# mworchel/svbrdf-estimation

Measured on AMD Instinct MI355X. Metric: rendered 256x256 patches/sec (fwd+bwd rendering loss), higher is better.
Workload: dtype f32

## Files before the change

### svbrdf_estimation_amd/csrc/svbrdf_kernels.hip

```cpp

#include <hip/hip_runtime.h>

#include <atomic>
#include <cstdint>
#include <cstdio>
#include <cstdlib>
#include <cmath>
#include <cstring>

#include "svbrdf_hip.h"

#ifndef SVBRDF_TU
#define SVBRDF_TU 2
#endif
#define SVBRDF_TU_MAIN (SVBRDF_TU == 0 || SVBRDF_TU == 2)
#define SVBRDF_TU_ADJOINT_PLAIN (SVBRDF_TU == 1 || SVBRDF_TU == 2)
#define SVBRDF_TU_ADJOINT_EXTRA (SVBRDF_TU == 3 || SVBRDF_TU == 2)
#define SVBRDF_TU_AUX (SVBRDF_TU == 4)

namespace {

constexpr int kThreads = 256;
constexpr int kLossThreads = 256;
constexpr float kPi = 3.14159274101257324219f;
constexpr float kMinDot = 0.001f;
constexpr float kMinRough = 0.001f;


__device__ __forceinline__ float dot3(float ax, float ay, float az, float bx, float by, float bz)
{
    const float p0 = ax * bx, p1 = ay * by, p2 = az * bz;
    return (p0 + p1) + p2;
}

__device__ __forceinline__ float fma_(float a, float b, float c) { return __builtin_fmaf(a, b, c); }
__device__ __forceinline__ float rcp_(float x) { return __builtin_amdgcn_rcpf(x); }
__device__ __forceinline__ float rsq_(float x) { return __builtin_amdgcn_rsqf(x); }
__device__ __forceinline__ float log2_(float x) { return __builtin_amdgcn_logf(x); }

#ifndef SVBRDF_SCALE_BLOCKS
#define SVBRDF_SCALE_BLOCKS 1024
#endif
#ifndef SVBRDF_TIMING
#define SVBRDF_TIMING 0
#endif
#ifndef SVBRDF_K3_MIN_WAVES
#define SVBRDF_K3_MIN_WAVES 4
#endif

struct Recip {
    float b, y;
};
__device__ __forceinline__ float div_rn(float a, const Recip &r)
{
    const float q = a * r.y;
    return fma_(fma_(-r.b, q, a), r.y, q);
}

__device__ __forceinline__ Recip length_rn(float x, float &seed)
{
    const float y = rsq_(x);
    const float g = x * y;
    seed = y;
    const float len = fma_(fma_(-g, g, x), 0.5f * y, g);
    const float e = fma_(-len, y, 1.0f);
    return Recip{len, fma_(e, y, y)};
}

struct VConst {
    float tiny;
    float pi, inv_pi;
    float ln2;
    float huge;
};
__device__ __forceinline__ float vreg(float c)
{
    asm volatile("" : "+v"(c));
    return c;
}
__device__ __forceinline__ VConst make_vconst()
{
    return VConst{vreg(kMinDot), vreg(kPi), vreg(1.0f / kPi), vreg(0.693147180559945309417f), vreg(1.0e30f)};
}


struct Geom {
    float wox, woy, woz;
    float wix, wiy, wiz;
    float hx, hy, hz;
    float p;
    float E[3];
};

__device__ __forceinline__ Geom geometry(const VConst &K, const float sc[9], float x, float y)
{
    Geom g;
    const float rcx = sc[0] - x, rcy = sc[1] - y, rcz = sc[2];
    const float rlx = sc[3] - x, rly = sc[4] - y, rlz = sc[5];
    float yc, yl, yh;
    const Recip ic = length_rn(dot3(rcx, rcy, rcz, rcx, rcy, rcz), yc);
    const Recip il = length_rn(dot3(rlx, rly, rlz, rlx, rly, rlz), yl);
    g.wox = div_rn(rcx, ic); g.woy = div_rn(rcy, ic); g.woz = div_rn(rcz, ic);
    g.wix = div_rn(rlx, il); g.wiy = div_rn(rly, il); g.wiz = div_rn(rlz, il);
    const float sx = g.wix + g.wox, sy = g.wiy + g.woy, sz = g.wiz + g.woz;
    const Recip ih = length_rn(dot3(sx, sy, sz, sx, sy, sz), yh);
    g.hx = div_rn(sx, ih); g.hy = div_rn(sy, ih); g.hz = div_rn(sz, ih);
    const float VH = fmaxf(fma_(g.wox, g.hx, fma_(g.woy, g.hy, g.woz * g.hz)), K.tiny);
    const float t = 1.0f - VH;
    const float t2 = t * t;
    g.p = (t2 * t2) * t;
    const float fall = yl * yl;
#pragma unroll
    for (int k = 0; k < 3; ++k) g.E[k] = sc[6 + k] * fall;
    return g;
}

struct Maps {
    float n[3], d[3], r[3], s[3];
};

struct Grad {
    float n[3], d[3], r[3], s[3];
};

struct MapK {
    float n[3];
    float A[3];
    float oA[3];
    float s[3], oms[3];
    float dpi[3];
    float r4m[3];
};

template <bool BWD>
__device__ __forceinline__ MapK prepare(const Maps &m)
{
    MapK k;
    constexpr float inv_pi = 1.0f / kPi;
#pragma unroll
    for (int c = 0; c < 3; ++c) {
        const float r = fmaxf(m.r[c], kMinRough);
        const float a = r * r;
        k.n[c] = m.n[c];
        k.A[c] = a * a;
        k.oA[c] = 1.0f - k.A[c];
        k.s[c] = m.s[c];
        k.oms[c] = 1.0f - m.s[c];
        k.dpi[c] = m.d[c] * inv_pi;
        if (BWD) k.r4m[c] = (m.r[c] >= kMinRough) ? 4.0f * (a * r) : 0.0f;
    }
    return k;
}

__device__ __forceinline__ bool tied_roughness(const Maps &m) { return m.r[0] == m.r[1] && m.r[1] == m.r[2]; }

struct Dots {
    float nh_raw, vn_raw, ln_raw;
    float NH, NH2, oN;
    float VN, LN;
    float VN2, LN2;
    float LNp;
};

__device__ __forceinline__ Dots dots(const VConst &K, const Geom &g, const MapK &m)
{
    Dots d;
    d.nh_raw = dot3(m.n[0], m.n[1], m.n[2], g.hx, g.hy, g.hz);
    d.vn_raw = fma_(g.wox, m.n[0], fma_(g.woy, m.n[1], g.woz * m.n[2]));
    d.ln_raw = fma_(g.wix, m.n[0], fma_(g.wiy, m.n[1], g.wiz * m.n[2]));
    d.NH = fmaxf(d.nh_raw, K.tiny);
    d.VN = fmaxf(d.vn_raw, K.tiny);
    d.LN = fmaxf(d.ln_raw, K.tiny);
    d.LNp = fmaxf(d.ln_raw, 0.0f);
    d.NH2 = d.NH * d.NH;
    d.oN = 1.0f - d.NH2;
    d.VN2 = d.VN * d.VN;
    d.LN2 = d.LN * d.LN;
    return d;
}

struct Lobe {
    float GD, KA, KV, KL, KN;
};

template <bool BWD>
__device__ __forceinline__ Lobe lobe(const VConst &K, float A, float oA, const Dots &d)
{
    Lobe l;
    const float yV = fma_(d.VN2, oA, A), yL = fma_(d.LN2, oA, A);
    const float iV = rsq_(yV), iL = rsq_(yL);
    const float sV = yV * iV, sL = yL * iL;
    const float PV = d.VN + sV, PL = d.LN + sL;
    const float PP = PV * PL;
    const float den_raw = fma_(d.NH2, A, d.oN);
    const float den = fmaxf(den_raw, K.tiny);
    const float pd = K.pi * den;
    const float Q = pd * den;
    const float R = rcp_(PP * Q);
    l.GD = A * R;
    if (BWD) {
        const float RQ = R * Q;
        const float tV = (RQ * PL) * l.GD;
        const float tL = (RQ * PV) * l.GD;
        l.KV = -tV * fma_(d.VN * oA, iV, 1.0f);
        l.KL = -tL * fma_(d.LN * oA, iL, 1.0f);
        const float Kden = (den_raw >= K.tiny) ? (-2.0f * l.GD) * ((R * PP) * pd) : 0.0f;
        const float hV = (1.0f - d.VN2) * iV, hL = (1.0f - d.LN2) * iL;
        l.KA = fma_(-0.5f, fma_(tV, hV, tL * hL), fma_(Kden, d.NH2, R));
        l.KN = -Kden * oA;
    }
    return l;
}

template <int NL, bool BWD>
__device__ __forceinline__ void shade(const VConst &K, const Geom &g, const MapK &m, const Dots &d, Lobe lb[NL],
                                      float F[3], float f[3], float rad[3])
{
#pragma unroll
    for (int l = 0; l < NL; ++l) lb[l] = lobe<BWD>(K, m.A[l], m.oA[l], d);
#pragma unroll
    for (int k = 0; k < 3; ++k) {
        F[k] = fma_(m.oms[k], g.p, m.s[k]);
        f[k] = fma_(F[k], lb[NL == 3 ? k : 0].GD - m.dpi[k], m.dpi[k]);
        rad[k] = f[k] * (g.E[k] * d.LNp);
    }
}

template <int NL, bool DEFER_D = false, bool DEFER_R = false>
__device__ __forceinline__ void shade_bwd(const VConst &K, const Geom &g, const MapK &m, const Dots &d, const Lobe lb[NL],
                                          const float F[3], const float f[3], const float g_rad[3], Grad &acc)
{
    float g_LNp, W[NL];
    const float inv_pi = K.inv_pi;
    const float omp = 1.0f - g.p;
#pragma unroll
    for (int k = 0; k < 3; ++k) {
        const Lobe &l = lb[NL == 3 ? k : 0];
        const float gE = g_rad[k] * g.E[k];
        const float g_f = gE * d.LNp;
        g_LNp = k == 0 ? gE * f[k] : fma_(gE, f[k], g_LNp);
        const float g_F = g_f * (l.GD - m.dpi[k]);
        acc.s[k] = fma_(g_F, omp, acc.s[k]);
        acc.d[k] = DEFER_D ? fma_(g_f, 1.0f - F[k], acc.d[k]) : fma_(g_f * (1.0f - F[k]), inv_pi, acc.d[k]);
        const float gGD = g_f * F[k];
        acc.r[k] = DEFER_R ? fma_(gGD, l.KA, acc.r[k]) : fma_(gGD * l.KA, m.r4m[k], acc.r[k]);
        if (NL == 3 || k == 0) W[NL == 3 ? k : 0] = gGD;
        else W[0] += gGD;
    }
    float g_VN = W[0] * lb[0].KV, g_LN = W[0] * lb[0].KL, sN = W[0] * lb[0].KN;
#pragma unroll
    for (int l = 1; l < NL; ++l) {
        g_VN = fma_(W[l], lb[l].KV, g_VN);
        g_LN = fma_(W[l], lb[l].KL, g_LN);
        sN = fma_(W[l], lb[l].KN, sN);
    }
    float g_NH = (sN * 2.0f) * d.NH;
    if (!(d.nh_raw >= K.tiny)) g_NH = 0.0f;
    if (!(d.vn_raw >= K.tiny)) g_VN = 0.0f;
    if (!(d.ln_raw >= K.tiny)) g_LN = 0.0f;
    if (!(d.ln_raw >= 0.0f)) g_LNp = 0.0f;
    const float gl = g_LN + g_LNp;
    acc.n[0] = fma_(g_NH, g.hx, fma_(g_VN, g.wox, fma_(gl, g.wix, acc.n[0])));
    acc.n[1] = fma_(g_NH, g.hy, fma_(g_VN, g.woy, fma_(gl, g.wiy, acc.n[1])));
    acc.n[2] = fma_(g_NH, g.hz, fma_(g_VN, g.woz, fma_(gl, g.wiz, acc.n[2])));
}


typedef float vec2f __attribute__((ext_vector_type(2)));
typedef float vec4f __attribute__((ext_vector_type(4)));
template <int VEC> struct VecT;
template <> struct VecT<1> { using type = float; };
template <> struct VecT<2> { using type = vec2f; };
template <> struct VecT<4> { using type = vec4f; };

template <int VEC, bool NT = false>
__device__ __forceinline__ void load_vec(const float *__restrict__ p, float out[VEC])
{
    using V = typename VecT<VEC>::type;
    const V v = NT ? __builtin_nontemporal_load(reinterpret_cast<const V *>(p)) : *reinterpret_cast<const V *>(p);
    const float *f = reinterpret_cast<const float *>(&v);
#pragma unroll
    for (int i = 0; i < VEC; ++i) out[i] = f[i];
}

template <int VEC, bool NT = false>
__device__ __forceinline__ void store_vec(float *__restrict__ p, const float in[VEC])
{
    using V = typename VecT<VEC>::type;
    V v;
    float *f = reinterpret_cast<float *>(&v);
#pragma unroll
    for (int i = 0; i < VEC; ++i) f[i] = in[i];
    if (NT) __builtin_nontemporal_store(v, reinterpret_cast<V *>(p));
    else *reinterpret_cast<V *>(p) = v;
}

template <int VEC, bool NT = false>
__device__ __forceinline__ void load_maps(const float *__restrict__ base, size_t plane, size_t pix,
                                          Maps m[VEC])
{
#pragma unroll
    for (int k = 0; k < 3; ++k) {
        float t[VEC];
        load_vec<VEC, NT>(base + (size_t)(0 + k) * plane + pix, t);
#pragma unroll
        for (int v = 0; v < VEC; ++v) m[v].n[k] = t[v];
        load_vec<VEC, NT>(base + (size_t)(3 + k) * plane + pix, t);
#pragma unroll
        for (int v = 0; v < VEC; ++v) m[v].d[k] = t[v];
        load_vec<VEC, NT>(base + (size_t)(6 + k) * plane + pix, t);
#pragma unroll
        for (int v = 0; v < VEC; ++v) m[v].r[k] = t[v];
        load_vec<VEC, NT>(base + (size_t)(9 + k) * plane + pix, t);
#pragma unroll
        for (int v = 0; v < VEC; ++v) m[v].s[k] = t[v];
    }
}

template <int VEC, bool NT = false>
__device__ __forceinline__ void store_grads(float *__restrict__ base, size_t plane, size_t pix,
                                            const Grad g[VEC])
{
#pragma unroll
    for (int k = 0; k < 3; ++k) {
        float t[VEC];
#pragma unroll
        for (int v = 0; v < VEC; ++v) t[v] = g[v].n[k];
        store_vec<VEC, NT>(base + (size_t)(0 + k) * plane + pix, t);
#pragma unroll
        for (int v = 0; v < VEC; ++v) t[v] = g[v].d[k];
        store_vec<VEC, NT>(base + (size_t)(3 + k) * plane + pix, t);
#pragma unroll
        for (int v = 0; v < VEC; ++v) t[v] = g[v].r[k];
        store_vec<VEC, NT>(base + (size_t)(6 + k) * plane + pix, t);
#pragma unroll
        for (int v = 0; v < VEC; ++v) t[v] = g[v].s[k];
        store_vec<VEC, NT>(base + (size_t)(9 + k) * plane + pix, t);
    }
}

#ifndef SVBRDF_K3_STORE_AUX
#define SVBRDF_K3_STORE_AUX 17
#endif
#ifndef SVBRDF_K3_LOAD_AUX
#define SVBRDF_K3_LOAD_AUX 0
#endif
struct PlaneBuf {
    __amdgpu_buffer_rsrc_t rsrc;
    unsigned lane_bytes;
    unsigned plane_bytes;
};
__device__ __forceinline__ PlaneBuf plane_buf(const float *item_base, int planes, size_t plane, size_t pix)
{
    PlaneBuf p;
    p.rsrc = __builtin_amdgcn_make_buffer_rsrc(const_cast<float *>(item_base), 0, (int)(planes * plane * sizeof(float)),
                                               0x00020000);
    p.lane_bytes = (unsigned)pix * 4u;
    p.plane_bytes = (unsigned)plane * 4u;
    return p;
}
__device__ __forceinline__ float plane_load(const PlaneBuf &p, int k)
{
    return __builtin_bit_cast(float, __builtin_amdgcn_raw_buffer_load_b32(p.rsrc, p.lane_bytes, k * p.plane_bytes, SVBRDF_K3_LOAD_AUX));
}
__device__ __forceinline__ void plane_store(const PlaneBuf &p, int k, float v)
{
    __builtin_amdgcn_raw_buffer_store_b32(__builtin_bit_cast(unsigned, v), p.rsrc, p.lane_bytes, k * p.plane_bytes,
                                          SVBRDF_K3_STORE_AUX);
}

__device__ __forceinline__ void load_maps_k3(const float *__restrict__ base, size_t plane, size_t pix, Maps &m)
{
    const PlaneBuf p = plane_buf(base, 12, plane, pix);
#pragma unroll
    for (int k = 0; k < 3; ++k) {
        m.n[k] = plane_load(p, 0 + k);
        m.d[k] = plane_load(p, 3 + k);
        m.r[k] = plane_load(p, 6 + k);
        m.s[k] = plane_load(p, 9 + k);
    }
}

__device__ __forceinline__ void store_grads_k3(float *__restrict__ base, size_t plane, size_t pix, const Grad &g)
{
    const PlaneBuf p = plane_buf(base, 12, plane, pix);
#pragma unroll
    for (int k = 0; k < 3; ++k) {
        plane_store(p, 0 + k, g.n[k]);
        plane_store(p, 3 + k, g.d[k]);
        plane_store(p, 6 + k, g.r[k]);
        plane_store(p, 9 + k, g.s[k]);
    }
}

__device__ __forceinline__ void zero_grad(Grad &g)
{
// ... 158 lines not shown

template <int VEC>
__global__ __launch_bounds__(kThreads) void k_render_fwd(const float *__restrict__ maps,
                                                         const float *__restrict__ scenes,
                                                         const float *__restrict__ xrow,
                                                         float *__restrict__ out, const int *__restrict__ offsets,
                                                         int shared, int S, int H, int W)
{
    render_fwd_body<VEC>(maps, scenes, xrow, out, offsets, shared != 0, S, H, W);
}

template <int VEC>
__global__ __launch_bounds__(kThreads) void k_render_fwd_inl([[maybe_unused]] const SceneBlock table,
                                                             const float *__restrict__ maps,
                                                             const float *__restrict__ xrow, float *__restrict__ out,
                                                             int shared, int S, int H, int W)
{
    const float *__restrict__ rows = (const float *)__builtin_amdgcn_kernarg_segment_ptr();
    render_fwd_body<VEC>(maps, rows, xrow, out, nullptr, shared != 0, S, H, W);
}

#ifndef SVBRDF_PHOTO_MIN_WAVES
#define SVBRDF_PHOTO_MIN_WAVES 4
#endif
#define SVBRDF_PHOTO_ATTRS __attribute__((amdgpu_waves_per_eu(SVBRDF_PHOTO_MIN_WAVES, 8)))
struct PhotoBlock {
    float v[SVBRDF_HOST_SCENES_MAX_ROWS * 9];
    float sigma[SVBRDF_HOST_SCENES_MAX_ROWS];
};

template <int VEC, int EPI>
__global__ __launch_bounds__(kThreads) SVBRDF_PHOTO_ATTRS void k_render_inputs(const float *__restrict__ maps,
                                                            const float *__restrict__ scenes,
                                                            const float *__restrict__ sigma, PhiloxKey key,
                                                            const float *__restrict__ xrow, float *__restrict__ out,
                                                            int S, int H, int W)
{
    render_fwd_body<VEC, EPI>(maps, scenes, xrow, out, nullptr, false, S, H, W, Epilogue{sigma, key});
}

template <int VEC, int EPI>
__global__ __launch_bounds__(kThreads) SVBRDF_PHOTO_ATTRS void k_render_inputs_inl([[maybe_unused]] const PhotoBlock table, PhiloxKey key,
                                                                const float *__restrict__ maps,
                                                                const float *__restrict__ xrow, float *__restrict__ out,
                                                                int S, int H, int W)
{
    const float *__restrict__ rows = (const float *)__builtin_amdgcn_kernarg_segment_ptr();
    render_fwd_body<VEC, EPI>(maps, rows, xrow, out, nullptr, false, S, H, W,
                              Epilogue{rows + SVBRDF_HOST_SCENES_MAX_ROWS * 9, key});
}

template <int VEC, int NL>
__device__ __forceinline__ void render_bwd_loop(const MapK mk[VEC], const float x[VEC], float y,
                                                const float *__restrict__ scp, const float *__restrict__ go,
                                                size_t plane, int S, Grad acc[VEC])
{
    const VConst K = make_vconst();
    for (int s = 0; s < S; ++s, scp += 9, go += 3 * plane) {
        float sc[9];
        load_scene(scp, sc);
        float gr[3][VEC];
#pragma unroll
        for (int k = 0; k < 3; ++k) load_vec<VEC, true>(go + (size_t)k * plane, gr[k]);
#pragma unroll
        for (int v = 0; v < VEC; ++v) {
            const Geom g = geometry(K, sc, x[v], y);
            const Dots d = dots(K, g, mk[v]);
            Lobe lb[NL];
            float F[3], f[3], rad[3];
            shade<NL, true>(K, g, mk[v], d, lb, F, f, rad);
            const float g_rad[3] = {gr[0][v], gr[1][v], gr[2][v]};
            shade_bwd<NL>(K, g, mk[v], d, lb, F, f, g_rad, acc[v]);
        }
    }
}

template <int VEC>
__device__ __forceinline__ void render_bwd_body(const float *__restrict__ maps, const float *__restrict__ scenes,
                                                const float *__restrict__ xrow, const float *__restrict__ grad_out,
                                                float *__restrict__ grad_maps, const int *__restrict__ offsets,
                                                bool shared, int S, int H, int W)
{
    const size_t plane = (size_t)H * W;
    const size_t pix = ((size_t)blockIdx.x * kThreads + threadIdx.x) * VEC;
    const int b = blockIdx.y;
    if (pix >= plane) return;
    MapK mk[VEC];
    bool tied = true;
    {
        Maps m[VEC];
        load_maps<VEC, true>(maps + (size_t)b * 12 * plane, plane, pix, m);
#pragma unroll
        for (int v = 0; v < VEC; ++v) {
            mk[v] = prepare<true>(m[v]);
            tied = tied && tied_roughness(m[v]);
        }
    }
    float x[VEC], y;
    pixel_coords<VEC>(xrow, pix, W, x, y);
    Grad acc[VEC];
#pragma unroll
    for (int v = 0; v < VEC; ++v) zero_grad(acc[v]);
    size_t first = (size_t)b * S;
    if (offsets) {
        first = (size_t)offsets[b];
        S = offsets[b + 1] - offsets[b];
    }
    const float *__restrict__ scp = scenes + (shared ? 0 : first * 9);
    const float *__restrict__ go = grad_out + first * 3 * plane + pix;
    if (__all(tied)) render_bwd_loop<VEC, 1>(mk, x, y, scp, go, plane, S, acc);
    else render_bwd_loop<VEC, 3>(mk, x, y, scp, go, plane, S, acc);
    store_grads<VEC, true>(grad_maps + (size_t)b * 12 * plane, plane, pix, acc);
}

template <int VEC>
__global__ __launch_bounds__(kThreads) void k_render_bwd(const float *__restrict__ maps,
                                                         const float *__restrict__ scenes,
                                                         const float *__restrict__ xrow,
                                                         const float *__restrict__ grad_out,
                                                         float *__restrict__ grad_maps, const int *__restrict__ offsets,
                                                         int shared, int S, int H, int W)
{
    render_bwd_body<VEC>(maps, scenes, xrow, grad_out, grad_maps, offsets, shared != 0, S, H, W);
}

template <int VEC>
__global__ __launch_bounds__(kThreads) void k_render_bwd_inl([[maybe_unused]] const SceneBlock table,
                                                             const float *__restrict__ maps,
                                                             const float *__restrict__ xrow,
                                                             const float *__restrict__ grad_out,
                                                             float *__restrict__ grad_maps, int shared, int S, int H, int W)
{
    const float *__restrict__ rows = (const float *)__builtin_amdgcn_kernarg_segment_ptr();
    render_bwd_body<VEC>(maps, rows, xrow, grad_out, grad_maps, nullptr, shared != 0, S, H, W);
}

__device__ __forceinline__ float wave_sum(float v)
{
#pragma unroll
    for (int off = 32; off > 0; off >>= 1) v += __shfl_xor(v, off, 64);
    return v;
}

constexpr int kLossSlots = 64;
constexpr int kLossCountShift = 48;
constexpr unsigned long long kLossSumMask = (1ULL << kLossCountShift) - 1;
constexpr unsigned long long kLossTicketMask = 0xffffffffULL;
constexpr unsigned long long kLossNonFiniteFlag = 1ULL << 32;

template <int NL, bool WITH_GRAD, int DEFER = 0>
__device__ __forceinline__ void loss_pixel_scene(const VConst &K, const Geom &g, const MapK &mi,
                                                 const MapK &mt, float eps, float inv_count, float &lsum, Grad &acc)
{
    float rt[3];
    {
        const Dots dt = dots(K, g, mt);
        Lobe lt[NL];
        float Ft[3], ft[3];
        shade<NL, false>(K, g, mt, dt, lt, Ft, ft, rt);
    }
    const Dots di = dots(K, g, mi);
    Lobe li[NL];
    float Fi[3], fi[3], ri[3], g_rad[3];
    shade<NL, WITH_GRAD>(K, g, mi, di, li, Fi, fi, ri);
    {
        constexpr float c = 9.765625e-04f;
        const float ec = eps * c, nc = inv_count * c;
        float b[3], bt[3], ib[3];
#pragma unroll
        for (int k = 0; k < 3; ++k) { b[k] = fma_(ri[k], c, ec); bt[k] = fma_(rt[k], c, ec); }
        {
            const float P = b[0] * b[1];
            const float r = rcp_(P * b[2]);
            const float t = r * b[2];
            ib[0] = t * b[1]; ib[1] = t * b[0]; ib[2] = r * P;
        }
#pragma unroll
        for (int k = 0; k < 3; ++k) {
            const float lg = (b[k] != bt[k]) ? log2_(bt[k] * ib[k]) : 0.0f;
            lsum += fabsf(lg);
            const float mag = (lg != 0.0f) ? nc * ib[k] : 0.0f;
            g_rad[k] = -__builtin_bit_cast(float, __builtin_bit_cast(unsigned, mag) | (__builtin_bit_cast(unsigned, lg) & 0x80000000u));
        }
    }
    if (WITH_GRAD) shade_bwd<NL, (DEFER & 1) != 0, (DEFER & 2) != 0>(K, g, mi, di, li, Fi, fi, g_rad, acc);
}

template <bool WITH_GRAD, int DEFER = 0>
__device__ __forceinline__ void loss_pixel_scene_by_channel(const VConst &K, const Geom &g, const MapK &mi, const MapK &mt,
                                                            float eps, float inv_count, float &lsum, Grad &acc)
{
    const Dots dt = dots(K, g, mt);
    const Dots di = dots(K, g, mi);
    constexpr float c = 9.765625e-04f;
    const float ec = eps * c, nc = inv_count * c;
    const float omp = 1.0f - g.p;
    float g_LNp = 0.0f, g_VN = 0.0f, g_LN = 0.0f, sN = 0.0f;
#pragma unroll
    for (int k = 0; k < 3; ++k) {
        const Lobe lt = lobe<false>(K, mt.A[k], mt.oA[k], dt);
        const float Ft = fma_(mt.oms[k], g.p, mt.s[k]);
        const float ft = fma_(Ft, lt.GD - mt.dpi[k], mt.dpi[k]);
        const float rt = ft * (g.E[k] * dt.LNp);
        const Lobe li = lobe<WITH_GRAD>(K, mi.A[k], mi.oA[k], di);
        const float Fi = fma_(mi.oms[k], g.p, mi.s[k]);
        const float fi = fma_(Fi, li.GD - mi.dpi[k], mi.dpi[k]);
        const float ri = fi * (g.E[k] * di.LNp);
        const float b = fma_(ri, c, ec), bt = fma_(rt, c, ec);
        const float ib = rcp_(b);
        const float lg = (b != bt) ? log2_(bt * ib) : 0.0f;
        lsum += fabsf(lg);
        if (WITH_GRAD) {
            const float mag = (lg != 0.0f) ? nc * ib : 0.0f;
            const float g_rad = -__builtin_bit_cast(float, __builtin_bit_cast(unsigned, mag) | (__builtin_bit_cast(unsigned, lg) & 0x80000000u));
            const float gE = g_rad * g.E[k];
            const float g_f = gE * di.LNp;
            g_LNp = fma_(gE, fi, g_LNp);
            const float g_F = g_f * (li.GD - mi.dpi[k]);
            acc.s[k] = fma_(g_F, omp, acc.s[k]);
            acc.d[k] = (DEFER & 1) ? fma_(g_f, 1.0f - Fi, acc.d[k]) : fma_(g_f * (1.0f - Fi), K.inv_pi, acc.d[k]);
            const float gGD = g_f * Fi;
            acc.r[k] = (DEFER & 2) ? fma_(gGD, li.KA, acc.r[k]) : fma_(gGD * li.KA, mi.r4m[k], acc.r[k]);
            g_VN = fma_(gGD, li.KV, g_VN);
            g_LN = fma_(gGD, li.KL, g_LN);
            sN = fma_(gGD, li.KN, sN);
        }
    }
    if (WITH_GRAD) {
        float g_NH = (sN * 2.0f) * di.NH;
        if (!(di.nh_raw >= K.tiny)) g_NH = 0.0f;
        if (!(di.vn_raw >= K.tiny)) g_VN = 0.0f;
        if (!(di.ln_raw >= K.tiny)) g_LN = 0.0f;
        if (!(di.ln_raw >= 0.0f)) g_LNp = 0.0f;
        const float gl = g_LN + g_LNp;
        acc.n[0] = fma_(g_NH, g.hx, fma_(g_VN, g.wox, fma_(gl, g.wix, acc.n[0])));
        acc.n[1] = fma_(g_NH, g.hy, fma_(g_VN, g.woy, fma_(gl, g.wiy, acc.n[1])));
        acc.n[2] = fma_(g_NH, g.hz, fma_(g_VN, g.woz, fma_(gl, g.wiz, acc.n[2])));
    }
}

template <int NL, bool WITH_GRAD, int DEFER = 0>
__device__ __forceinline__ void loss_pixel_scene_any(const VConst &K, const Geom &g, const MapK &mi, const MapK &mt,
                                                     float eps, float inv_count, float &lsum, Grad &acc)
{
    if (NL == 3)
        loss_pixel_scene_by_channel<WITH_GRAD, DEFER>(K, g, mi, mt, eps, inv_count, lsum, acc);
    else
        loss_pixel_scene<NL, WITH_GRAD, DEFER>(K, g, mi, mt, eps, inv_count, lsum, acc);
}

#ifndef SVBRDF_K3_STAGGER
#define SVBRDF_K3_STAGGER 64
#endif
#ifndef SVBRDF_K3_EARLY_COORDS
#define SVBRDF_K3_EARLY_COORDS 1
#endif
template <int NL, bool WITH_GRAD, int DEFER = 0>
__device__ __forceinline__ float loss_scene_loop(const MapK &mi, const MapK &mt_in, float x, float y,
                                                 const float *__restrict__ scp, const float *sc_lds, int S,
                                                 float eps, float inv_count, Grad &acc)
{
    constexpr int ST = 9;
    float lsum = 0.0f;
    const VConst K = make_vconst();
    eps = vreg(eps);
    inv_count = vreg(inv_count);
    float sc[9];
#if SVBRDF_TIMING
    const long long tm0 = clock64(), wc0 = wall_clock64();
#endif
    if (WITH_GRAD) {
        load_scene(scp, sc);
        Geom ga = geometry(K, sc, x, y), gb;
        load_scene(scp + (S > 1 ? ST : 0), sc);
#define SVBRDF_K3_PASS(G_CUR, G_NEXT, SI)                                                                             \
        {                                                                                                          \
            asm volatile("" ::"s"(sc[0]), "s"(sc[8]));            \
            float cur[9];                                                                                          \
            _Pragma("unroll") for (int i = 0; i < 9; ++i) cur[i] = sc[i];                                          \
            load_scene(scp + ((SI) + 2 < S ? 2 * ST : ((SI) + 1 < S ? ST : 0)), sc);                               \
            scp += ((SI) + 1 < S) ? ST : 0;                                                                        \
            __builtin_amdgcn_sched_barrier(0);                                                                     \
                                                    \
            G_NEXT = geometry(K, cur, x, y);                      \
            loss_pixel_scene_any<NL, WITH_GRAD, DEFER>(K, G_CUR, mi, mt_in, eps, inv_count, lsum, acc);                   \
        }
        for (int s = 0;;) {
            SVBRDF_K3_PASS(ga, gb, s)
            if (++s >= S) break;
            SVBRDF_K3_PASS(gb, ga, s)
            if (++s >= S) break;
        }
#undef SVBRDF_K3_PASS
    } else {
        load_scene(sc_lds, sc);
        Geom g_next = geometry(K, sc, x, y);
        for (int s = 0; s < S; ++s) {
            const Geom g = g_next;
            load_scene(sc_lds + (s + 1 < S ? s + 1 : s) * 9, sc);
            g_next = geometry(K, sc, x, y);
            loss_pixel_scene_any<NL, WITH_GRAD, DEFER>(K, g, mi, mt_in, eps, inv_count, lsum, acc);
        }
    }
    lsum *= 0.693147180559945309417f;
    if (WITH_GRAD && DEFER) {
#pragma unroll
        for (int k = 0; k < 3; ++k) {
            if (DEFER & 1) acc.d[k] *= K.inv_pi;
            if (DEFER & 2) acc.r[k] *= mi.r4m[k];
        }
    }
#if SVBRDF_TIMING
    if (WITH_GRAD) {
        acc.n[0] = (float)(clock64() - tm0);
        acc.n[1] = (float)(wall_clock64() - wc0);
        acc.n[2] = (float)(wc0 & 0xffffff);
    }
#endif
    return lsum;
}

struct L1Params {
    float sum_scale;
    float grad_scale;
    float eps;
};

__device__ __forceinline__ float signed_scale(float delta, float scale)
{
    return __builtin_amdgcn_fmed3f(delta * 1.0e30f, -1.0f, 1.0f) * scale;
}

struct Head {
    float nx, ny, nz;
    float inv_len;
};

__device__ __forceinline__ Head decode_head(const float e[9], Maps &m)
{
    Head h;
    const float vx = e[0] * 3.0f, vy = e[1] * 3.0f;
    float seed;
    const Recip il = length_rn((vx * vx + vy * vy) + 1.0f, seed);
    h.nx = div_rn(vx, il); h.ny = div_rn(vy, il); h.nz = div_rn(1.0f, il);
    h.inv_len = il.y;
    m.n[0] = h.nx; m.n[1] = h.ny; m.n[2] = h.nz;
    const float r = (e[5] + 1.0f) * 0.5f;
#pragma unroll
    for (int k = 0; k < 3; ++k) {
        m.d[k] = (e[2 + k] + 1.0f) * 0.5f;
        m.r[k] = r;
        m.s[k] = (e[6 + k] + 1.0f) * 0.5f;
    }
    return h;
}

__device__ __forceinline__ void head_bwd(const Head &h, const Grad &g, float ge[9])
{
    const float ng = fma_(h.nx, g.n[0], fma_(h.ny, g.n[1], h.nz * g.n[2]));
    ge[0] = 3.0f * (fma_(-h.nx, ng, g.n[0]) * h.inv_len);
    ge[1] = 3.0f * (fma_(-h.ny, ng, g.n[1]) * h.inv_len);
#pragma unroll
    for (int k = 0; k < 3; ++k) {
        ge[2 + k] = 0.5f * g.d[k];
        ge[6 + k] = 0.5f * g.s[k];
    }
    ge[5] = 0.5f * ((g.r[0] + g.r[1]) + g.r[2]);
}

__device__ __forceinline__ bool loss_arrive(float t, float fixed_scale, unsigned long long *__restrict__ ws)
{
    const unsigned nblocks = gridDim.x * gridDim.y, bid = blockIdx.y * gridDim.x + blockIdx.x;
    const unsigned slot = bid & (kLossSlots - 1);
    const unsigned slot_blocks = (nblocks - slot + kLossSlots - 1) / kLossSlots;
    const float scaled = fma_(t, fixed_scale, 0.5f);
    const float limit = 140737488355328.0f * 0.999f * rcp_((float)slot_blocks);
    const bool finite = scaled >= 0.0f && scaled < limit;
    const unsigned long long fixed = finite ? (unsigned long long)scaled : 0ULL;
    if (!finite) {
        atomicOr(&ws[kLossSlots], kLossNonFiniteFlag);
        __threadfence();
    }
    const unsigned long long old = atomicAdd(&ws[slot], (1ULL << kLossCountShift) | fixed);
    if ((unsigned)(old >> kLossCountShift) + 1 == slot_blocks) {
        const unsigned nslots = nblocks < (unsigned)kLossSlots ? nblocks : (unsigned)kLossSlots;
        const unsigned long long ticket = atomicAdd(&ws[kLossSlots], 1ULL);
        if ((unsigned)(ticket & kLossTicketMask) + 1 == nslots) return true;
    }
    return false;
}

__device__ __forceinline__ void loss_finish(unsigned lane, unsigned long long *__restrict__ ws, float *__restrict__ loss_out,
                                            double loss_scale)
{
    const unsigned nblocks = gridDim.x * gridDim.y;
    unsigned long long v = 0;
    if (lane < (unsigned)kLossSlots && lane < nblocks) v = atomicExch(&ws[lane], 0ULL) & kLossSumMask;
#pragma unroll
    for (int off = 32; off > 0; off >>= 1) v += __shfl_xor(v, off, 64);
    if (lane == 0) {
        __threadfence();
        const unsigned long long tail = atomicExch(&ws[kLossSlots], 0ULL);
        loss_out[0] = (tail & kLossNonFiniteFlag) ? __builtin_nanf("") : (float)((double)v * loss_scale);
    }
}

template <bool HEAD>
__device__ __forceinline__ void store_pixel_grad(const Head &head, const Grad &acc, float *__restrict__ grad_input, int b,
                                                 size_t plane, size_t pix)
{
    if (HEAD) {
        float ge[9];
        head_bwd(head, acc, ge);
        float *__restrict__ gp = grad_input + (size_t)b * 9 * plane;
        const PlaneBuf pb = plane_buf(gp, 9, plane, pix);
#pragma unroll
        for (int k = 0; k < 9; ++k) plane_store(pb, k, ge[k]);
    } else {
        store_grads_k3(grad_input + (size_t)b * 12 * plane, plane, pix, acc);
    }
}

template <bool WITH_GRAD, bool WITH_L1, bool HEAD, bool EARLY_COORDS = false>
__device__ __forceinline__ void rendering_loss_body(const float *__restrict__ input, const float *__restrict__ target,
                                                    const float *__restrict__ scenes, const float *__restrict__ xrow,
                                                    float eps, float inv_count, double loss_scale, float fixed_scale,
                                                    L1Params l1, float *__restrict__ grad_input,
                                                    unsigned long long *__restrict__ ws, float *__restrict__ loss_out,
                                                    int S, int H, int W)
{
    extern __shared__ __attribute__((aligned(16))) float sc_lds[];
    constexpr float kLn2 = 0.693147180559945309417f;
    const size_t plane = (size_t)H * W;
    const size_t pix = (size_t)blockIdx.x * kLossThreads + threadIdx.x;
    const int b = blockIdx.y;
    const bool active = pix < plane;
    float lsum = 0.0f;
    Grad acc;
    Head head;
#if SVBRDF_TIMING
    const long long t_entry = wall_clock64();
#endif
#if SVBRDF_K3_STAGGER
    if (WITH_GRAD && EARLY_COORDS && S >= 6) {
        const unsigned layer = (blockIdx.y * gridDim.x + blockIdx.x) >> 8;
        if (layer == 1) __builtin_amdgcn_s_sleep(SVBRDF_K3_STAGGER);
        else if (layer == 2) { __builtin_amdgcn_s_sleep(SVBRDF_K3_STAGGER); __builtin_amdgcn_s_sleep(SVBRDF_K3_STAGGER); }
        else if (layer == 3) { __builtin_amdgcn_s_sleep(SVBRDF_K3_STAGGER); __builtin_amdgcn_s_sleep(SVBRDF_K3_STAGGER); __builtin_amdgcn_s_sleep(SVBRDF_K3_STAGGER); }
    }
#endif
    if (!WITH_GRAD) {
        for (int i = threadIdx.x; i < S * 9; i += kLossThreads) sc_lds[i] = scenes[(size_t)b * S * 9 + i];
        __syncthreads();
    }
    if (active) {
        Maps in[1], tg[1];
        [[maybe_unused]] float x_early = 0.0f, y_early = 0.0f;
        const bool early_coords = SVBRDF_K3_EARLY_COORDS && EARLY_COORDS && WITH_GRAD && (W & (W - 1)) == 0;
        if (early_coords) {
            const unsigned p32 = (unsigned)pix, sh = (unsigned)__builtin_ctz((unsigned)W);
            x_early = xrow[p32 & (unsigned)(W - 1)];
            y_early = xrow[p32 >> sh];
            __builtin_amdgcn_sched_barrier(0);
        }
        if (HEAD) {
            float e[9];
            const float *__restrict__ ip = input + (size_t)b * 9 * plane;
            const PlaneBuf pb = plane_buf(ip, 9, plane, pix);
#pragma unroll
            for (int k = 0; k < 9; ++k) e[k] = plane_load(pb, k);
            head = decode_head(e, in[0]);
        } else {
            load_maps_k3(input + (size_t)b * 12 * plane, plane, pix, in[0]);
        }
        load_maps_k3(target + (size_t)b * 12 * plane, plane, pix, tg[0]);
        zero_grad(acc);
        float l1sum = 0.0f;
        constexpr int kDefer = WITH_GRAD ? (WITH_L1 ? 1 : 3) : 0;
        if (WITH_L1) {
            float a[6], b[6], ia[6];
#pragma unroll
            for (int k = 0; k < 3; ++k) {
                a[k] = in[0].d[k] + l1.eps; b[k] = tg[0].d[k] + l1.eps;
                a[3 + k] = in[0].s[k] + l1.eps; b[3 + k] = tg[0].s[k] + l1.eps;
            }
            {
                float pre[6];
                pre[0] = a[0];
#pragma unroll
                for (int k = 1; k < 6; ++k) pre[k] = pre[k - 1] * a[k];
                float r = rcp_(pre[5]);
#pragma unroll
                for (int k = 5; k > 0; --k) { ia[k] = r * pre[k - 1]; r *= a[k]; }
                ia[0] = r;
            }
#pragma unroll
            for (int k = 0; k < 3; ++k) {
                const float dn = in[0].n[k] - tg[0].n[k], dr = in[0].r[k] - tg[0].r[k];
                const float dd = (a[k] == b[k]) ? 0.0f : -kLn2 * log2_(b[k] * ia[k]);
                const float ds = (a[3 + k] == b[3 + k]) ? 0.0f : -kLn2 * log2_(b[3 + k] * ia[3 + k]);
                l1sum += (fabsf(dn) + fabsf(dr)) + (fabsf(dd) + fabsf(ds));
                if (WITH_GRAD) {
                    acc.n[k] = signed_scale(dn, l1.grad_scale);
                    acc.r[k] = signed_scale(dr, l1.grad_scale);
                    acc.d[k] = signed_scale(dd, l1.grad_scale) * ia[k];
                    if (kDefer & 1) acc.d[k] *= kPi;
                    acc.s[k] = signed_scale(ds, l1.grad_scale) * ia[3 + k];
                }
            }
        }
        const bool tied = tied_roughness(in[0]) && tied_roughness(tg[0]);
        const MapK mi = prepare<WITH_GRAD>(in[0]), mt = prepare<false>(tg[0]);
        float x[1], y;
        if (early_coords) {
            x[0] = x_early;
            y = -y_early;
        } else if ((W & (W - 1)) == 0) {
            const unsigned p32 = (unsigned)pix, sh = (unsigned)__builtin_ctz((unsigned)W);
            x[0] = xrow[p32 & (unsigned)(W - 1)];
            y = -xrow[p32 >> sh];
        } else {
            pixel_coords<1>(xrow, pix, W, x, y);
        }
        {
            const float chk = (((in[0].n[0] + in[0].n[1]) + (in[0].n[2] + in[0].r[0])) + (in[0].r[1] + in[0].r[2])) +
                              (((tg[0].n[0] + tg[0].n[1]) + (tg[0].n[2] + tg[0].r[0])) + (tg[0].r[1] + tg[0].r[2]));
            x[0] += chk - chk;
        }
        const float *__restrict__ scp = scenes + (size_t)b * S * 9;
        if (__all(tied))
            lsum = loss_scene_loop<1, WITH_GRAD, kDefer>(mi, mt, x[0], y, scp, sc_lds, S, eps, inv_count, acc);
        else
            lsum = loss_scene_loop<3, WITH_GRAD, kDefer>(mi, mt, x[0], y, scp, sc_lds, S, eps, inv_count, acc);
        if (WITH_L1) lsum = fma_(l1sum, l1.sum_scale, lsum);
#if SVBRDF_TIMING
        if (WITH_GRAD && !HEAD) {
            acc.d[0] = (float)(t_entry & 0xffffff);
            acc.d[1] = (float)(wall_clock64() & 0xffffff);
            const unsigned hw = __builtin_amdgcn_s_getreg((31 << 11) | 4), xcc = __builtin_amdgcn_s_getreg((3 << 11) | 20);
            acc.d[2] = (float)(((xcc & 15u) << 8) | (((hw >> 13) & 7u) << 5) | (((hw >> 12) & 1u) << 4) | ((hw >> 8) & 15u));
        }
#endif
        if (WITH_GRAD) store_pixel_grad<HEAD>(head, acc, grad_input, b, plane, pix);
    }
    {
        __shared__ float wave_part[kLossThreads / 64];
        __shared__ int finisher;
        lsum = wave_sum(lsum);
        if ((threadIdx.x & 63) == 0) wave_part[threadIdx.x >> 6] = lsum;
        __syncthreads();
        if (threadIdx.x == 0) {
            float t = 0.0f;
#pragma unroll
            for (int w = 0; w < kLossThreads / 64; ++w) t += wave_part[w];
            finisher = loss_arrive(t, fixed_scale, ws) ? 1 : 0;
        }
        __syncthreads();
        if (finisher && threadIdx.x < 64) loss_finish(threadIdx.x, ws, loss_out, loss_scale);
    }
}

#define SVBRDF_K3_ATTRS __launch_bounds__(kLossThreads) __attribute__((amdgpu_waves_per_eu(SVBRDF_K3_MIN_WAVES, 8)))

template <bool WITH_GRAD, bool WITH_L1, bool HEAD>
__global__ SVBRDF_K3_ATTRS void k_rendering_loss(const float *__restrict__ input, const float *__restrict__ target,
                                                 const float *__restrict__ scenes, const float *__restrict__ xrow,
                                                 float eps, float inv_count, double loss_scale, float fixed_scale,
                                                 L1Params l1, float *__restrict__ grad_input,
                                                 unsigned long long *__restrict__ ws, float *__restrict__ loss_out,
                                                 int S, int H, int W)
{
    rendering_loss_body<WITH_GRAD, WITH_L1, HEAD>(input, target, scenes, xrow, eps, inv_count, loss_scale, fixed_scale,
                                                  l1, grad_input, ws, loss_out, S, H, W);
}

template <bool WITH_GRAD, bool WITH_L1, bool HEAD>
__global__ SVBRDF_K3_ATTRS void k_rendering_loss_inl([[maybe_unused]] const SceneBlock table,
                                                     const float *__restrict__ input, const float *__restrict__ target,
                                                     const float *__restrict__ xrow, float eps, float inv_count,
                                                     double loss_scale, float fixed_scale, L1Params l1,
                                                     float *__restrict__ grad_input, unsigned long long *__restrict__ ws,
                                                     float *__restrict__ loss_out, int S, int H, int W)
{
    const float *__restrict__ rows = (const float *)__builtin_amdgcn_kernarg_segment_ptr();
    rendering_loss_body<WITH_GRAD, WITH_L1, HEAD, true>(input, target, rows, xrow, eps, inv_count, loss_scale,
                                                           fixed_scale, l1, grad_input, ws, loss_out, S, H, W);
}


#if defined(SVBRDF_ISA_PROBE)
extern "C" __global__ void svbrdf_isa_probe_dot3(const float *__restrict__ a, float *__restrict__ o)
{
    o[threadIdx.x] = dot3(a[threadIdx.x], a[threadIdx.x + 64], a[threadIdx.x + 128], a[threadIdx.x + 192], a[threadIdx.x + 256],
                          a[threadIdx.x + 320]);
}
#endif

#if SVBRDF_TU_MAIN
__global__ __launch_bounds__(kThreads) void k_scale_inplace(float *__restrict__ data, const float *__restrict__ scale,
                                                            size_t n)
{
    const float s = scale[0];
    if (s == 1.0f) return;
    const size_t stride = (size_t)gridDim.x * kThreads;
    for (size_t i = (size_t)blockIdx.x * kThreads + threadIdx.x; i < n; i += stride) data[i] *= s;
}

__device__ __forceinline__ unsigned hash32(unsigned x)
{
    x ^= x >> 16; x *= 0x7feb352dU; x ^= x >> 15; x *= 0x846ca68bU; x ^= x >> 16;
    return x;
}

__global__ __launch_bounds__(kThreads) void k_check_arith(unsigned long long n, unsigned seed, float lo, float hi,
                                                          unsigned long long *__restrict__ counts)
{
    unsigned long long bad_div = 0, bad_sqrt = 0;
    const unsigned long long stride = (unsigned long long)gridDim.x * kThreads;
    for (unsigned long long i = (unsigned long long)blockIdx.x * kThreads + threadIdx.x; i < n; i += stride) {
        const unsigned h0 = hash32((unsigned)i * 2654435761U + seed), h1 = hash32(h0 ^ (unsigned)(i >> 32) ^ 0x9e3779b9U);
        const float u0 = (float)(h0 >> 8) * (1.0f / 16777216.0f), u1 = (float)(h1 >> 8) * (1.0f / 16777216.0f);
        const float b = lo * exp2f(u0 * log2f(hi / lo));
        const float a = (2.0f * u1 - 1.0f) * hi;
        float seed;
        const Recip r = length_rn(b, seed);
        const float len = sqrtf(b);
        if (r.b != len) ++bad_sqrt;
        if (div_rn(a, r) != a / len) ++bad_div;
    }
    if (bad_div) atomicAdd(&counts[0], bad_div);
    if (bad_sqrt) atomicAdd(&counts[1], bad_sqrt);
}

template <int VEC>
__global__ __launch_bounds__(kThreads) void k_mix_materials(const float *__restrict__ m0, const float *__restrict__ m1,
                                                            const float *__restrict__ alpha, float *__restrict__ out,
                                                            size_t plane)
{
    const size_t pix = ((size_t)blockIdx.x * kThreads + threadIdx.x) * VEC;
    const int b = blockIdx.y;
    if (pix >= plane) return;
    const float a = alpha[b], oma = 1.0f - a;
    const float *__restrict__ p0 = m0 + (size_t)b * 12 * plane + pix;
    const float *__restrict__ p1 = m1 + (size_t)b * 12 * plane + pix;
    float *__restrict__ po = out + (size_t)b * 12 * plane + pix;
    float n0[3][VEC], n1[3][VEC], nm[3][VEC];
#pragma unroll
    for (int k = 0; k < 3; ++k) {
        load_vec<VEC, true>(p0 + (size_t)k * plane, n0[k]);
        load_vec<VEC, true>(p1 + (size_t)k * plane, n1[k]);
    }
#pragma unroll
    for (int v = 0; v < VEC; ++v) {
        const float z0 = fmaxf(0.01f, n0[2][v]), z1 = fmaxf(0.01f, n1[2][v]);
#pragma unroll
        for (int k = 0; k < 3; ++k) nm[k][v] = a * (n0[k][v] / z0) + oma * (n1[k][v] / z1);
        const float len = sqrtf((nm[0][v] * nm[0][v] + nm[1][v] * nm[1][v]) + nm[2][v] * nm[2][v]);
#pragma unroll
        for (int k = 0; k < 3; ++k) nm[k][v] = nm[k][v] / len;
    }
#pragma unroll
    for (int k = 0; k < 3; ++k) store_vec<VEC, true>(po + (size_t)k * plane, nm[k]);
#pragma unroll
    for (int k = 3; k < 12; ++k) {
        float x0[VEC], x1[VEC], y[VEC];
        load_vec<VEC, true>(p0 + (size_t)k * plane, x0);
        load_vec<VEC, true>(p1 + (size_t)k * plane, x1);
#pragma unroll
        for (int v = 0; v < VEC; ++v) y[v] = a * x0[v] + oma * x1[v];
        store_vec<VEC, true>(po + (size_t)k * plane, y);
    }
}

__global__ __launch_bounds__(64) void k_clock_probe(unsigned long long *__restrict__ out, unsigned long long ticks)
{
    if (threadIdx.x != 0) return;
    const unsigned long long r0 = wall_clock64(), c0 = clock64();
    unsigned long long r1 = r0;
    while (r1 - r0 < ticks) {
        __builtin_amdgcn_s_sleep(32);
        r1 = wall_clock64();
    }
    const unsigned long long c1 = clock64();
    out[0] = c1 - c0;
    out[1] = r1 - r0;
}
// ... 508 lines not shown
```

Measured before the change: 216,600.

## Trim per-scene ALU in rendering loss via algebraic folding and deferred scaling

Rewrites the geometry Fresnel term to compute 1-VH directly from the half-vector length, folds the loss scale constant into the light falloff via ldexp, and fuses radiance computation with the log-loss bias into a single FMA. The loss gradient sign/magnitude selection becomes a single med3 clamp. A new defer mode accumulates diffuse gradients without the per-scene (1-F) factor and rescales once after the loop. Together these aim to cut VALU instructions in the inner per-scene loop, at the cost of small floating-point rounding differences and reliance on algebraic identities (e.g. VH = |s|/2) that hold only for normalized vectors.

```diff
diff --git a/svbrdf_estimation_amd/csrc/svbrdf_kernels.hip b/svbrdf_estimation_amd/csrc/svbrdf_kernels.hip
--- a/svbrdf_estimation_amd/csrc/svbrdf_kernels.hip
+++ b/svbrdf_estimation_amd/csrc/svbrdf_kernels.hip
@@ -83,6 +83,8 @@
     return VConst{vreg(kMinDot), vreg(kPi), vreg(1.0f / kPi), vreg(0.693147180559945309417f), vreg(1.0e30f)};
 }
 
+constexpr int kLossScaleExp = -10;
+
 
 struct Geom {
     float wox, woy, woz;
@@ -92,7 +94,8 @@
     float E[3];
 };
 
-__device__ __forceinline__ Geom geometry(const VConst &K, const float sc[9], float x, float y)
+template <bool LOSS = false>
+__device__ __forceinline__ Geom geometry([[maybe_unused]] const VConst &K, const float sc[9], float x, float y)
 {
     Geom g;
     const float rcx = sc[0] - x, rcy = sc[1] - y, rcz = sc[2];
@@ -105,11 +108,10 @@
     const float sx = g.wix + g.wox, sy = g.wiy + g.woy, sz = g.wiz + g.woz;
     const Recip ih = length_rn(dot3(sx, sy, sz, sx, sy, sz), yh);
     g.hx = div_rn(sx, ih); g.hy = div_rn(sy, ih); g.hz = div_rn(sz, ih);
-    const float VH = fmaxf(fma_(g.wox, g.hx, fma_(g.woy, g.hy, g.woz * g.hz)), K.tiny);
-    const float t = 1.0f - VH;
+    const float t = fminf(fma_(-0.5f, ih.b, 1.0f), 1.0f - kMinDot);
     const float t2 = t * t;
     g.p = (t2 * t2) * t;
-    const float fall = yl * yl;
+    const float fall = LOSS ? __builtin_amdgcn_ldexpf(yl * yl, kLossScaleExp) : yl * yl;
 #pragma unroll
     for (int k = 0; k < 3; ++k) g.E[k] = sc[6 + k] * fall;
     return g;
@@ -183,14 +185,14 @@
     float GD, KA, KV, KL, KN;
 };
 
-template <bool BWD>
+template <bool BWD, bool FUSE_PX = true>
 __device__ __forceinline__ Lobe lobe(const VConst &K, float A, float oA, const Dots &d)
 {
     Lobe l;
     const float yV = fma_(d.VN2, oA, A), yL = fma_(d.LN2, oA, A);
     const float iV = rsq_(yV), iL = rsq_(yL);
-    const float sV = yV * iV, sL = yL * iL;
-    const float PV = d.VN + sV, PL = d.LN + sL;
+    const float PV = FUSE_PX ? fma_(yV, iV, d.VN) : d.VN + yV * iV;
+    const float PL = FUSE_PX ? fma_(yL, iL, d.LN) : d.LN + yL * iL;
     const float PP = PV * PL;
     const float den_raw = fma_(d.NH2, A, d.oN);
     const float den = fmaxf(den_raw, K.tiny);
@@ -213,8 +215,8 @@
 }
 
 template <int NL, bool BWD>
-__device__ __forceinline__ void shade(const VConst &K, const Geom &g, const MapK &m, const Dots &d, Lobe lb[NL],
-                                      float F[3], float f[3], float rad[3])
+__device__ __forceinline__ void brdf(const VConst &K, const Geom &g, const MapK &m, const Dots &d, Lobe lb[NL],
+                                     float F[3], float f[3])
 {
 #pragma unroll
     for (int l = 0; l < NL; ++l) lb[l] = lobe<BWD>(K, m.A[l], m.oA[l], d);
@@ -222,11 +224,33 @@
     for (int k = 0; k < 3; ++k) {
         F[k] = fma_(m.oms[k], g.p, m.s[k]);
         f[k] = fma_(F[k], lb[NL == 3 ? k : 0].GD - m.dpi[k], m.dpi[k]);
-        rad[k] = f[k] * (g.E[k] * d.LNp);
-    }
-}
-
-template <int NL, bool DEFER_D = false, bool DEFER_R = false>
+    }
+}
+
+template <int NL, bool BWD>
+__device__ __forceinline__ void shade(const VConst &K, const Geom &g, const MapK &m, const Dots &d, Lobe lb[NL],
+                                      float F[3], float f[3], float rad[3])
+{
+    brdf<NL, BWD>(K, g, m, d, lb, F, f);
+#pragma unroll
+    for (int k = 0; k < 3; ++k) rad[k] = f[k] * (g.E[k] * d.LNp);
+}
+
+template <int NL, bool BWD>
+__device__ __forceinline__ void shade_loss(const VConst &K, const Geom &g, const MapK &m, const Dots &d, Lobe lb[NL],
+                                           float F[3], float f[3], float ec, float b[3])
+{
+    brdf<NL, BWD>(K, g, m, d, lb, F, f);
+#pragma unroll
+    for (int k = 0; k < 3; ++k) b[k] = fma_(f[k], g.E[k] * d.LNp, ec);
+}
+
+__device__ __forceinline__ float loss_grad_of_b(const VConst &K, float lg, float M)
+{
+    return __builtin_amdgcn_fmed3f(-lg * K.huge, -M, M);
+}
+
+template <int NL, bool DEFER_D = false, bool DEFER_R = false, bool DEFER_S = false>
 __device__ __forceinline__ void shade_bwd(const VConst &K, const Geom &g, const MapK &m, const Dots &d, const Lobe lb[NL],
                                           const float F[3], const float f[3], const float g_rad[3], Grad &acc)
 {
@@ -239,9 +263,15 @@
         const float gE = g_rad[k] * g.E[k];
         const float g_f = gE * d.LNp;
         g_LNp = k == 0 ? gE * f[k] : fma_(gE, f[k], g_LNp);
-        const float g_F = g_f * (l.GD - m.dpi[k]);
-        acc.s[k] = fma_(g_F, omp, acc.s[k]);
-        acc.d[k] = DEFER_D ? fma_(g_f, 1.0f - F[k], acc.d[k]) : fma_(g_f * (1.0f - F[k]), inv_pi, acc.d[k]);
+        if (DEFER_S) {
+            const float gfo = g_f * omp;
+            acc.s[k] = fma_(gfo, l.GD - m.dpi[k], acc.s[k]);
+            acc.d[k] += gfo;
+        } else {
+            const float g_F = g_f * (l.GD - m.dpi[k]);
+            acc.s[k] = fma_(g_F, omp, acc.s[k]);
+            acc.d[k] = DEFER_D ? fma_(g_f, 1.0f - F[k], acc.d[k]) : fma_(g_f * (1.0f - F[k]), inv_pi, acc.d[k]);
+        }
         const float gGD = g_f * F[k];
         acc.r[k] = DEFER_R ? fma_(gGD, l.KA, acc.r[k]) : fma_(gGD * l.KA, m.r4m[k], acc.r[k]);
         if (NL == 3 || k == 0) W[NL == 3 ? k : 0] = gGD;
@@ -706,23 +736,20 @@
 __device__ __forceinline__ void loss_pixel_scene(const VConst &K, const Geom &g, const MapK &mi,
                                                  const MapK &mt, float eps, float inv_count, float &lsum, Grad &acc)
 {
-    float rt[3];
+    const float ec = __builtin_amdgcn_ldexpf(eps, kLossScaleExp);
+    float bt[3];
     {
         const Dots dt = dots(K, g, mt);
         Lobe lt[NL];
         float Ft[3], ft[3];
-        shade<NL, false>(K, g, mt, dt, lt, Ft, ft, rt);
+        shade_loss<NL, false>(K, g, mt, dt, lt, Ft, ft, ec, bt);
     }
     const Dots di = dots(K, g, mi);
     Lobe li[NL];
-    float Fi[3], fi[3], ri[3], g_rad[3];
-    shade<NL, WITH_GRAD>(K, g, mi, di, li, Fi, fi, ri);
+    float Fi[3], fi[3], b[3], g_rad[3];
+    shade_loss<NL, WITH_GRAD>(K, g, mi, di, li, Fi, fi, ec, b);
     {
-        constexpr float c = 9.765625e-04f;
-        const float ec = eps * c, nc = inv_count * c;
-        float b[3], bt[3], ib[3];
-#pragma unroll
-        for (int k = 0; k < 3; ++k) { b[k] = fma_(ri[k], c, ec); bt[k] = fma_(rt[k], c, ec); }
+        float ib[3];
         {
             const float P = b[0] * b[1];
             const float r = rcp_(P * b[2]);
@@ -733,11 +760,10 @@
         for (int k = 0; k < 3; ++k) {
             const float lg = (b[k] != bt[k]) ? log2_(bt[k] * ib[k]) : 0.0f;
             lsum += fabsf(lg);
-            const float mag = (lg != 0.0f) ? nc * ib[k] : 0.0f;
-            g_rad[k] = -__builtin_bit_cast(float, __builtin_bit_cast(unsigned, mag) | (__builtin_bit_cast(unsigned, lg) & 0x80000000u));
-        }
-    }
-    if (WITH_GRAD) shade_bwd<NL, (DEFER & 1) != 0, (DEFER & 2) != 0>(K, g, mi, di, li, Fi, fi, g_rad, acc);
+            g_rad[k] = loss_grad_of_b(K, lg, inv_count * ib[k]);
+        }
+    }
+    if (WITH_GRAD) shade_bwd<NL, (DEFER & 1) != 0, (DEFER & 2) != 0, (DEFER & 4) != 0>(K, g, mi, di, li, Fi, fi, g_rad, acc);
 }
 
 template <bool WITH_GRAD, int DEFER = 0>
@@ -746,33 +772,35 @@
 {
     const Dots dt = dots(K, g, mt);
     const Dots di = dots(K, g, mi);
-    constexpr float c = 9.765625e-04f;
-    const float ec = eps * c, nc = inv_count * c;
+    const float ec = __builtin_amdgcn_ldexpf(eps, kLossScaleExp);
     const float omp = 1.0f - g.p;
     float g_LNp = 0.0f, g_VN = 0.0f, g_LN = 0.0f, sN = 0.0f;
 #pragma unroll
     for (int k = 0; k < 3; ++k) {
-        const Lobe lt = lobe<false>(K, mt.A[k], mt.oA[k], dt);
+        const Lobe lt = lobe<false, false>(K, mt.A[k], mt.oA[k], dt);
         const float Ft = fma_(mt.oms[k], g.p, mt.s[k]);
         const float ft = fma_(Ft, lt.GD - mt.dpi[k], mt.dpi[k]);
-        const float rt = ft * (g.E[k] * dt.LNp);
-        const Lobe li = lobe<WITH_GRAD>(K, mi.A[k], mi.oA[k], di);
+        const float bt = fma_(ft, g.E[k] * dt.LNp, ec);
+        const Lobe li = lobe<WITH_GRAD, false>(K, mi.A[k], mi.oA[k], di);
         const float Fi = fma_(mi.oms[k], g.p, mi.s[k]);
         const float fi = fma_(Fi, li.GD - mi.dpi[k], mi.dpi[k]);
-        const float ri = fi * (g.E[k] * di.LNp);
-        const float b = fma_(ri, c, ec), bt = fma_(rt, c, ec);
+        const float b = fma_(fi, g.E[k] * di.LNp, ec);
         const float ib = rcp_(b);
         const float lg = (b != bt) ? log2_(bt * ib) : 0.0f;
         lsum += fabsf(lg);
         if (WITH_GRAD) {
-            const float mag = (lg != 0.0f) ? nc * ib : 0.0f;
-            const float g_rad = -__builtin_bit_cast(float, __builtin_bit_cast(unsigned, mag) | (__builtin_bit_cast(unsigned, lg) & 0x80000000u));
-            const float gE = g_rad * g.E[k];
+            const float gE = loss_grad_of_b(K, lg, inv_count * ib) * g.E[k];
             const float g_f = gE * di.LNp;
             g_LNp = fma_(gE, fi, g_LNp);
-            const float g_F = g_f * (li.GD - mi.dpi[k]);
-            acc.s[k] = fma_(g_F, omp, acc.s[k]);
-            acc.d[k] = (DEFER & 1) ? fma_(g_f, 1.0f - Fi, acc.d[k]) : fma_(g_f * (1.0f - Fi), K.inv_pi, acc.d[k]);
+            if (DEFER & 4) {
+                const float gfo = g_f * omp;
+                acc.s[k] = fma_(gfo, li.GD - mi.dpi[k], acc.s[k]);
+                acc.d[k] += gfo;
+            } else {
+                const float g_F = g_f * (li.GD - mi.dpi[k]);
+                acc.s[k] = fma_(g_F, omp, acc.s[k]);
+                acc.d[k] = (DEFER & 1) ? fma_(g_f, 1.0f - Fi, acc.d[k]) : fma_(g_f * (1.0f - Fi), K.inv_pi, acc.d[k]);
+            }
             const float gGD = g_f * Fi;
             acc.r[k] = (DEFER & 2) ? fma_(gGD, li.KA, acc.r[k]) : fma_(gGD * li.KA, mi.r4m[k], acc.r[k]);
             g_VN = fma_(gGD, li.KV, g_VN);
@@ -825,7 +853,7 @@
 #endif
     if (WITH_GRAD) {
         load_scene(scp, sc);
-        Geom ga = geometry(K, sc, x, y), gb;
+        Geom ga = geometry<true>(K, sc, x, y), gb;
         load_scene(scp + (S > 1 ? ST : 0), sc);
 #define SVBRDF_K3_PASS(G_CUR, G_NEXT, SI)                                                                             \
         {                                                                                                          \
@@ -836,7 +864,7 @@
             scp += ((SI) + 1 < S) ? ST : 0;                                                                        \
             __builtin_amdgcn_sched_barrier(0);                                                                     \
                                                     \
-            G_NEXT = geometry(K, cur, x, y);                      \
+            G_NEXT = geometry<true>(K, cur, x, y);                \
             loss_pixel_scene_any<NL, WITH_GRAD, DEFER>(K, G_CUR, mi, mt_in, eps, inv_count, lsum, acc);                   \
         }
         for (int s = 0;;) {
@@ -848,11 +876,11 @@
 #undef SVBRDF_K3_PASS
     } else {
         load_scene(sc_lds, sc);
-        Geom g_next = geometry(K, sc, x, y);
+        Geom g_next = geometry<true>(K, sc, x, y);
         for (int s = 0; s < S; ++s) {
             const Geom g = g_next;
             load_scene(sc_lds + (s + 1 < S ? s + 1 : s) * 9, sc);
-            g_next = geometry(K, sc, x, y);
+            g_next = geometry<true>(K, sc, x, y);
             loss_pixel_scene_any<NL, WITH_GRAD, DEFER>(K, g, mi, mt_in, eps, inv_count, lsum, acc);
         }
     }
@@ -860,7 +888,8 @@
     if (WITH_GRAD && DEFER) {
 #pragma unroll
         for (int k = 0; k < 3; ++k) {
-            if (DEFER & 1) acc.d[k] *= K.inv_pi;
+            if (DEFER & 4) acc.d[k] *= mi.oms[k] * K.inv_pi;
+            else if (DEFER & 1) acc.d[k] *= K.inv_pi;
             if (DEFER & 2) acc.r[k] *= mi.r4m[k];
         }
     }
@@ -1030,7 +1059,7 @@
         load_maps_k3(target + (size_t)b * 12 * plane, plane, pix, tg[0]);
         zero_grad(acc);
         float l1sum = 0.0f;
-        constexpr int kDefer = WITH_GRAD ? (WITH_L1 ? 1 : 3) : 0;
+        constexpr int kDefer = WITH_GRAD ? (WITH_L1 ? 1 : 7) : 0;
         if (WITH_L1) {
             float a[6], b[6], ia[6];
 #pragma unroll
@@ -1085,7 +1114,7 @@
         if (__all(tied))
             lsum = loss_scene_loop<1, WITH_GRAD, kDefer>(mi, mt, x[0], y, scp, sc_lds, S, eps, inv_count, acc);
         else
-            lsum = loss_scene_loop<3, WITH_GRAD, kDefer>(mi, mt, x[0], y, scp, sc_lds, S, eps, inv_count, acc);
+            lsum = loss_scene_loop<3, WITH_GRAD, kDefer & 3>(mi, mt, x[0], y, scp, sc_lds, S, eps, inv_count, acc);
         if (WITH_L1) lsum = fma_(l1sum, l1.sum_scale, lsum);
 #if SVBRDF_TIMING
         if (WITH_GRAD && !HEAD) {
```

Measured after the change: 228,800, median of 6. 5.6% higher.
